# talmolab/sleap-nn

Hardware: AMD Instinct MI355X
Metric: frames/sec bottom-up UNet 1024x1024 inference (higher is better)
Workload: dtype f32

## Files before the change

sleap_nn_amd/csrc/model.hip:

```cpp
#include <algorithm>
#include <atomic>
#include <cmath>
#include <cstring>
#include <mutex>
#include <type_traits>
#include <vector>

#include "model_internal.h"
#include "train_kernels.h"

static constexpr size_t PH_PROBE_WORDS_PER_OP = 32768;

namespace ph {

static thread_local std::string g_err;

void set_error(const char* fmt, ...) {
  char buf[1024];
  va_list ap;
  va_start(ap, fmt);
  vsnprintf(buf, sizeof(buf), fmt, ap);
  va_end(ap);
  g_err = buf;
}
// ... 1174 lines not shown
        a.coutp = pad16(d.cout);
        a.B = batch;
        a.H = s0.h;
        a.W = s0.w;
        a.relu = (d.flags & PH_FLAG_RELU) ? 1 : 0;
        a.bn = op.bn;
        a.clock_probe = m->clock_probe ? m->clock_probe + PH_PROBE_WORDS_PER_OP * (op_index - 1) : nullptr;
        a.dst_pool = d.dst2 >= 0 ? slot_ptr(d.dst2) : nullptr;
        a.skip_dst = (a.dst_pool && plan.reuse && !plan.unread.empty() && plan.unread[d.dst]) ? 1 : 0;
        a.wpack_dma = op.w_dma_dev;
        a.wpack_wino = op.w_wino_dev;
        a.wpack_wino2 = op.w_wino2_dev;
        a.wpack_w16 = op.w_w16_dev;
        a.w16 = op.w16_dev;
        a.zeros = m->zeros_dev;
        apply_conv_options(m, a);
        a.wpack_sm = op.w_sm_dev;
        a.use_sm = m->conv_smallmap >= 2 ? 2 : ((m->conv_smallmap == 1 && m->conv_splitk == 1 && plan.reuse && m->use_dma) ? 1 : 0);
        a.wpack_wino4 = op.w_wino4_dev;
        a.use_wino4 = m->conv_wino4 == 3 ? 2 : ((m->conv_wino4 == 2 || (m->conv_wino4 == 1 && plan.reuse)) ? 1 : 0);
        if (op.w_n64_dev && op.w_wino2_dev && op.w_wino_dev && (m->conv_n32_wino2d >= 2 || (m->conv_n32_wino2d == 1 && plan.reuse)) && m->use_dma && m->conv_wino && m->conv_wino2d && m->conv_persist && !w16_fits(a) && wino2d_fits(a)) {
          a.bn = 64;
          a.wpack = op.w_n64_dev;
          a.bias = op.b_n64_dev;
          a.wpack_dma = nullptr;
        }
        if (a.splitk == 1 && !plan.reuse) a.splitk = 0;
        if (plan.tmp_bytes > 0) {
          a.split_scratch = reinterpret_cast<float*>(ws + plan.tmp_offset);
          a.split_scratch_bytes = plan.tmp_bytes;
        }
        if (deferred_up >= 0) {
          const ph_op_desc& up = m->ops[deferred_up].d;
          const SlotShape& sl = plan.slots[up.src0];
          ConvArgs f = a;
          f.src1 = slot_ptr(up.src0);
          f.src1_lowres = 1;
          if ((m->use_dma && conv3x3_dma_is_wino4(f)) || conv3x3_takes_sm(f)) {
            a = f;
          } else {
            rc = launch_upsample(slot_ptr(up.src0), slot_ptr(up.dst), batch, sl.h, sl.w, sl.cp, s);
            if (rc != PH_OK) return rc;
          }
          deferred_up = -1;
        }
        const bool on_sm = conv3x3_takes_sm(a);
        const double fill = (double)s0.h * s0.w / ((double)((s0.h + 15) / 16 * 16) * ((s0.w + 31) / 32 * 32));
        const double n_fill = (double)a.coutp / ((a.coutp + op.bn - 1) / op.bn * op.bn);
        const int bn_g = op.bn_g > 0 ? op.bn_g : 128;
        const double n_fill_g = (double)a.coutp / ((a.coutp + bn_g - 1) / bn_g * bn_g);
        double halo_gain = (op.w_wino_dev && m->use_dma) ? m->gemm_fill_threshold / m->gemm_fill_threshold_wino : 1.0;
        double halo_fill = fill;
        if (m->use_dma && m->conv_wino && m->conv_wino2d && m->conv_persist && op.w_wino2_dev && a.bn == 64 && a.c0p + a.c1p >= 32 && wino2d_fits(a)) {
          halo_fill = (double)s0.h * s0.w / ((double)((s0.h + 15) / 16 * 16) * ((s0.w + 15) / 16 * 16));
          halo_gain = m->gemm_fill_threshold / m->gemm_fill_threshold_wino2d;
        }
        if (!on_sm && m->use_dma && d.dst2 < 0 && op.w_gemm_dev && !a.src1_lowres && (halo_fill * halo_gain < m->gemm_fill_threshold || n_fill * halo_fill * halo_gain < 0.8 * n_fill_g)) {
          GemmArgs g{};
          g.src0 = a.src0;
          g.src1 = a.src1;
          g.c0p = a.c0p;
          g.c1p = a.c1p;
          g.wpack = op.w_gemm_dev;
          g.bias = op.b_gemm_dev;
          g.dst = a.dst;
          g.zeros = m->zeros_dev;
          g.coutp = a.coutp;
          g.bn = op.bn_g;
          g.M = batch * s0.h * s0.w;
          g.mode = 2;
          g.H = s0.h;
          g.W = s0.w;
          g.act = a.relu ? 1 : 0;
          g.late_split = m->gemm_late_split;
          g.persist2 = m->gemm_persist2;
          kv[op_index - 1] = PH_KV_ROWGEMM;
          rc = launch_gemm(g, s);
          break;
        }
        if (m->head_fuse && !a.dst_pool && ((a.coutp == 64 && a.bn == 64) || ((a.coutp == 16 || a.coutp == 32) && a.bn == 32)) && m->use_dma) {
          for (size_t j = op_index; j < m->ops.size(); ++j) {
            const ph_op_desc& hx = m->ops[j].d;
            if (hx.kind != PH_OP_HEAD || hx.src0 != d.dst) continue;
            ConvArgs no4 = a;
            no4.use_wino4 = 0;
            const bool on_w2d = a.coutp == 64 && hx.cout <= 32 && pad16(hx.cin0) == 64 && conv3x3_dma_is_wino2d(no4) && wino2d_ksplit(no4) <= 1;
            const bool on_w16 = a.coutp <= 32 && hx.cout <= 16 && pad16(hx.cin0) == a.coutp && conv3x3_dma_is_w16_head(a);
            const bool sm_head = on_sm && a.coutp <= 32 && pad16(hx.cin0) == a.coutp;
            if (!(hx.flags & PH_FLAG_SOFTMAX) && out_dev[hx.out_index] && (sm_head || (!on_sm && (on_w2d || on_w16)))) {
              a.head_w = m->ops[j].w_dev;
              a.head_b = m->ops[j].b_dev;
              a.head_dst = out_dev[hx.out_index];
              a.head_cout = hx.cout;
              a.head_wcp = a.coutp;
              a.head_sigmoid = (hx.flags & PH_FLAG_SIGMOID) ? 1 : 0;
              head_done[j] = 1;
              if (plan.reuse) {
                bool other = false;
                for (size_t k = 0; k < m->ops.size(); ++k)
                  if (k != j && (m->ops[k].d.src0 == d.dst || m->ops[k].d.src1 == d.dst)) other = true;
                if (!other) a.skip_dst = 1;
              }
            }
            break;
          }
        }
        if (m->pool_peephole && !a.dst_pool && !a.head_w && a.relu && m->use_dma && (a.bn == 64 || m->dma32) && op_index < m->ops.size()) {
          const ph_op_desc& nx = m->ops[op_index].d;
          if (nx.kind == PH_OP_POOL && nx.src0 == d.dst) {
            a.dst_pool = slot_ptr(nx.dst);
            if (conv3x3_dma_is_f2x2(a))
              pooled_by_conv = d.dst;
            else
              a.dst_pool = nullptr;
          }
        }
        if (on_sm) {
          kv[op_index - 1] = PH_KV_SMALLMAP;
          rc = launch_conv3x3_sm(a, s);
          break;
        }
        kv[op_index - 1] = (m->use_dma && (a.bn == 64 || m->dma32)) ? conv3x3_dma_variant(a) : PH_KV_DIRECT;
        rc = (m->use_dma && (a.bn == 64 || m->dma32)) ? launch_conv3x3_dma(a, s) : launch_conv3x3(a, s);
        break;
      }
      case PH_OP_POOL: {
        if (pooled_by_conv == d.src0) {
          pooled_by_conv = -1;
          break;
        }
        const SlotShape& s0 = plan.slots[d.src0];
        rc = fmt == FMT_F32 ? launch_pool(slot_ptr(d.src0), slot_ptr(d.dst), batch, s0.h, s0.w, s0.cp, s)
                            : launch_pool_fmt(fmt, slot_ptr(d.src0), slot_ptr(d.dst), batch, s0.h, s0.w, s0.cp, s);
        break;
      }
      case PH_OP_UPSAMPLE: {
        const SlotShape& s0 = plan.slots[d.src0];
        if (fmt == FMT_F32 && plan.reuse && m->upsample_fold && (m->conv_wino4 || m->conv_smallmap) && m->use_dma && op_index < m->ops.size()) {
          const PackedOp& nxo = m->ops[op_index];
          const ph_op_desc& nx = nxo.d;
          bool only = nx.kind == PH_OP_CONV && nx.ksize == 3 && nx.src1 == d.dst && nx.src0 != d.dst && nx.dst2 < 0 && ((m->conv_wino4 && nxo.w_wino4_dev != nullptr) || (m->conv_smallmap && nxo.w_sm_dev != nullptr));
          for (size_t k = 0; only && k < m->ops.size(); ++k)
            if (k != op_index && (m->ops[k].d.src0 == d.dst || m->ops[k].d.src1 == d.dst)) only = false;
          if (only) {
            deferred_up = (int)op_index - 1;
            break;
          }
        }
        if (fmt == FMT_F16 && plan.reuse && m->upsample_fold && m->conv_f16_rows && op_index < m->ops.size()) {
          const PackedOp& nxo = m->ops[op_index];
          const ph_op_desc& nx = nxo.d;
          bool only = nx.kind == PH_OP_CONV && nx.ksize == 3 && nx.src1 == d.dst && nx.src0 != d.dst && nxo.bn == 64 && plan.slots[nx.src0].h == 2 * s0.h && plan.slots[nx.src0].w == 2 * s0.w;
          for (size_t k = 0; only && k < m->ops.size(); ++k)
            if (k != op_index && (m->ops[k].d.src0 == d.dst || m->ops[k].d.src1 == d.dst)) only = false;
          if (only) {
            deferred_up = (int)op_index - 1;
            break;
          }
        }
        rc = fmt == FMT_F32 ? launch_upsample(slot_ptr(d.src0), slot_ptr(d.dst), batch, s0.h, s0.w, s0.cp, s)
                            : launch_upsample_fmt(fmt, slot_ptr(d.src0), slot_ptr(d.dst), batch, s0.h, s0.w, s0.cp, s, (fmt == FMT_F16 && m->upsample_f16math) ? 1 : 0);
        break;
      }
      case PH_OP_CONVT: {
        const SlotShape& s0 = plan.slots[d.src0];
        PH_REQUIRE(s0.c == d.cin0, "convT channel mismatch");
        if (fmt == FMT_F32 && m->convt_phase && op.wt_phase_dev[0]) {
          const SlotShape& so = plan.slots[d.dst];
          for (int ph = 0; ph < (m->convt_one_launch ? 1 : 4) && rc == PH_OK; ++ph) {
            GemmArgs g{};
            g.src0 = slot_ptr(d.src0);
            g.c0p = s0.cp;
// ... 448 lines not shown
```

sleap_nn_amd/csrc/net_kernels.hip:

```cpp
#include <type_traits>

#include "act_format.h"
#include "common.h"
#include "net_kernels.h"
#include "f16_kernels.h"

namespace ph {

typedef float f32x16 __attribute__((ext_vector_type(16)));
typedef float f32x4 __attribute__((ext_vector_type(4)));

constexpr int TH = 8, TW = 32, KC = 16, LROW = 20;
constexpr int HALO_W = TW + 2, HALO_H = TH + 2;

__device__ __forceinline__ void deal_tile(int id, int tiles, int nt_count, int* tile, int* ntile) {
  if ((tiles & 7) == 0) {
    const int xcd = id & 7, j = id >> 3;
    *ntile = j % nt_count;
    *tile = xcd * (tiles >> 3) + j / nt_count;
  } else {
    *ntile = id % nt_count;
    *tile = id / nt_count;
  }
}
// ... 1128 lines not shown
        if (a.accumulate) v += *d;
        *d = v;
      }
    }
    __syncthreads();
  }
}

static int cu_count(int* out);
static int launch_conv3x3_c16(const ConvArgs& a, hipStream_t s) {
  int n_cu = 0;
  const int rc = cu_count(&n_cu);
  if (rc != PH_OK) return rc;
  const int tiles = ((a.W + C16_TW - 1) / C16_TW) * ((a.H + C16_TH - 1) / C16_TH) * a.B;
  hipLaunchKernelGGL(conv3x3_c16_kernel, dim3(std::min(tiles, n_cu * 4)), dim3(256), 0, s, a);
  PH_HIP_CHECK(hipGetLastError());
  return PH_OK;
}

static int cu_count(int* out) { return device_cu_count(out); }

static int conv3x3_dma_route(const ConvArgs& a) {
  const bool wino = a.use_wino && a.wpack_wino && (a.bn == 64 || a.use_wino != 2);
  if (wino && a.persist && a.use_wino4 && a.c0p + a.c1p >= a.wino4_min_cin && wino4_fits(a)) return 4;
  if (wino && a.persist && a.use_w16 && w16_fits(a)) return 1;
  if (a.use_c16 && a.w16 && a.c0p == 16 && a.coutp == 16 && !a.src1 && !a.dst_pool) return 0;
  if (wino && a.persist && a.use_wino2d && a.wpack_wino2 && a.bn == 64 && a.c0p + a.c1p >= 32 && wino2d_fits(a)) return 2;
  return 3;
}
bool conv3x3_takes_sm(const ConvArgs& a) {
  if (!a.use_sm || !sm_fits(a)) return false;
  if (a.use_sm >= 2) return true;
  int n_cu = 0;
  if (device_cu_count(&n_cu) != PH_OK || n_cu <= 0) n_cu = 256;
  ConvArgs hi = a;
  hi.src1_lowres = 0;
  const int r = a.src1_lowres && conv3x3_dma_route(a) == 4 ? 4 : conv3x3_dma_route(hi);
  const double extra = (a.src1_lowres && r != 4) ? 6.0 : 0.0;
  const double Qn = (a.c0p + a.c1p) / 4.0;
  const long ntc = (a.coutp + 63) / 64;
  const bool may_split = a.split_scratch != nullptr;
  double other;
  if (r == 4) {
    const int ks = may_split ? wino4_ksplit_shape(a.B, a.H, a.W, a.c0p + a.c1p, a.coutp, a.splitk, n_cu) : 1;
    const long t4 = (long)((a.H + 15) / 16) * ((a.W + 31) / 32) * a.B * ntc;
    other = (double)((t4 * ks + n_cu - 1) / n_cu) * (11.0 + 1.5 * Qn / ks) + (ks > 1 ? 8.0 : 0.0);
  } else if (r == 2) {
    const int ks = may_split ? wino2d_ksplit_shape(a.B, a.H, a.W, a.c0p + a.c1p, a.coutp, a.splitk, n_cu) : 1;
    const long t2 = (long)((a.H + 15) / 16) * ((a.W + 15) / 16) * a.B * ntc;
    other = (double)((t2 * ks + n_cu - 1) / n_cu) * (8.0 + 1.0 * Qn / ks) + (ks > 1 ? 8.0 : 0.0);
  } else if (r == 1) {
    const long t1 = (long)((a.H + 31) / 32) * ((a.W + 15) / 16) * a.B;
    other = (double)((t1 + n_cu - 1) / n_cu) * (6.0 + 3.0 * (a.c0p + a.c1p) / 16.0);
  } else {
    return false;
  }
  if ((r == 4 || r == 2) && (a.coutp & 63) != 0 && (a.coutp & 63) <= 32) other *= 0.6;
  return sm_cost_us(a, n_cu) < other + extra;
}
bool conv3x3_dma_honours_mask(const ConvArgs& a) {
  const int r = conv3x3_dma_route(a);
  return (r == 1 || r == 2 || r == 4) && !a.dst_pool && !a.head_w && !a.skip_dst;
}
bool conv3x3_dma_is_f2x2(const ConvArgs& a) { const int r = conv3x3_dma_route(a); return r == 1 || r == 2; }
bool conv3x3_dma_is_wino2d(const ConvArgs& a) { return conv3x3_dma_route(a) == 2; }
bool conv3x3_dma_is_wino4(const ConvArgs& a) { return conv3x3_dma_route(a) == 4; }
bool conv3x3_dma_is_w16_head(const ConvArgs& a) { return conv3x3_dma_route(a) == 1 && w16_takes_head(a); }
int conv3x3_dma_variant(const ConvArgs& a) {
  switch (conv3x3_dma_route(a)) {
    case 0: return PH_KV_C16;
    case 1: return PH_KV_W16;
    case 2: return wino2d_ksplit(a) > 1 ? PH_KV_WINO2D_KS : PH_KV_WINO2D;
    case 4: return PH_KV_WINO4;
    default: break;
  }
  const bool wino = a.use_wino && a.wpack_wino && (a.bn == 64 || a.use_wino != 2);
  return (a.persist && wino) ? PH_KV_WINO1D : PH_KV_DIRECT;
}

int launch_conv3x3_dma(const ConvArgs& a, hipStream_t s) {
  const int route = conv3x3_dma_route(a);
  PH_REQUIRE(!a.relu_mask_src || ((route == 1 || route == 2 || route == 4) && !a.dst_pool && !a.head_w && !a.skip_dst),
             "relu_mask_src is applied by the F(2x2,3x3) / F(4x4,3x3) kernels' plain stores only (ask conv3x3_dma_honours_mask first)");
  PH_REQUIRE(!a.head_w || (route == 2 && !a.dst_pool && a.coutp == 64 && a.bn == 64 && a.head_cout >= 1 && a.head_cout <= 32 && a.head_wcp == 64 && a.head_b && a.head_dst) ||
                 (route == 1 && w16_takes_head(a) && a.head_cout >= 1 && a.head_cout <= 16 && a.head_wcp == a.coutp && a.head_b && a.head_dst),
             "a fused head needs the F(2x2,3x3) kernel on 64 output channels (<= 32 head channels) or the wave-private kernel on 16 -> 16 / 32 -> 32 channels (<= 16 head channels): ask conv3x3_dma_is_wino2d / _is_w16_head first");
  if (route == 1) return launch_conv3x3_w16(a, s);
  if (route == 0) return launch_conv3x3_c16(a, s);
  if (route == 2) return launch_conv3x3_wino2d(a, s);
  if (route == 4) return launch_conv3x3_wino4(a, s);
  PH_REQUIRE(!a.src1_lowres, "a half-resolution second source is only taken by the F(4x4,3x3) kernel (ask conv3x3_dma_is_wino4 first)");
  const int tiles = ((a.W + TW - 1) / TW) * ((a.H + D_TH - 1) / D_TH) * a.B;
  const int ntc = (a.coutp + a.bn - 1) / a.bn;
  const bool wino = a.use_wino && a.wpack_wino && (a.bn == 64 || a.use_wino != 2);
  int n_cu = 0;
  if (a.persist) {
    const int rc = cu_count(&n_cu);
    if (rc != PH_OK) return rc;
  }
  const dim3 grid_p(std::min(tiles * ntc, n_cu)), grid_1(tiles * ntc);
  const size_t lds_w = (size_t)(2 * D_A_PIECES + 3 * 12 * (a.bn / 32)) * 1024;
  const size_t lds_d = (size_t)2 * (D_A_PIECES + 9 * a.bn / 16) * 1024;
  if (a.bn == 64) {
    if (a.persist && wino)
      hipLaunchKernelGGL((conv3x3_wino_persist_kernel<64, 8>), grid_p, dim3(512), lds_w, s, a);
    else if (a.persist)
      hipLaunchKernelGGL(conv3x3_mfma_dma_persist_kernel<64>, grid_p, dim3(512), lds_d, s, a);
    else
      hipLaunchKernelGGL(conv3x3_mfma_dma_kernel<64>, grid_1, dim3(512), lds_d, s, a);
  } else {
    if (a.persist && wino)
      hipLaunchKernelGGL((conv3x3_wino_persist_kernel<32, 8>), grid_p, dim3(512), lds_w, s, a);
    else if (a.persist)
      hipLaunchKernelGGL(conv3x3_mfma_dma_persist_kernel<32>, grid_p, dim3(512), lds_d, s, a);
    else
      hipLaunchKernelGGL(conv3x3_mfma_dma_kernel<32>, grid_1, dim3(512), lds_d, s, a);
  }
  PH_HIP_CHECK(hipGetLastError());
  return PH_OK;
}

__device__ __forceinline__ void stem_store(const StemArgs& a, void* base, size_t pix, int c, float v) {
  if (a.out_fmt == FMT_SPLIT)
    store1<FMT_SPLIT>(base, pix, 16, c, v);
  else if (a.out_fmt == FMT_F16) {
    store1<FMT_F16>(base, pix, 32, c, v);
    store1<FMT_F16>(base, pix, 32, c + 16, 0.f);
  } else
    store1<FMT_F32>(base, pix, 16, c, v);
}

__device__ __forceinline__ void stem_store4(const StemArgs& a, void* base, size_t pix, int c0, const float (&v)[4]) {
  if (a.out_fmt == FMT_SPLIT)
    store4<FMT_SPLIT>(base, pix, 16, c0, v);
  else if (a.out_fmt == FMT_F16) {
    const float z[4] = {0.f, 0.f, 0.f, 0.f};
    store4<FMT_F16>(base, pix, 32, c0, v);
    store4<FMT_F16>(base, pix, 32, c0 + 16, z);
  } else
    store4<FMT_F32>(base, pix, 16, c0, v);
}

template <int CIN, int WINO>
__global__ __launch_bounds__(256, (CIN == 1 && WINO == 2) ? 5 : 4) void stem_fused_kernel(StemArgs a) {
  constexpr int IMG_W = TW + 4, IMG_H = TH + 4;
  __shared__ __attribute__((aligned(16))) float sA[HALO_H * HALO_W * LROW];
  __shared__ float sImg[CIN * IMG_H * IMG_W];
  __shared__ float sW0[9 * CIN * 16 + 16];

  const int tid = threadIdx.x;
  const int lane = tid & 63, wave = tid >> 6;
  const int tiles_x = (a.W + TW - 1) / TW, tiles_y = (a.H + TH - 1) / TH;
  const int per_xcd = (tiles_x * tiles_y * a.B + 7) >> 3;
  int t = (blockIdx.x & 7) * per_xcd + (blockIdx.x >> 3);
  if (t >= tiles_x * tiles_y * a.B) return;
  const int tx = t % tiles_x;
  t /= tiles_x;
  const int ty = t % tiles_y;
  const int b = t / tiles_y;
  const int x0 = tx * TW, y0 = ty * TH;

  for (int i = tid; i < CIN * IMG_H * IMG_W; i += 256) {
    const int c = i / (IMG_H * IMG_W), r = i - c * (IMG_H * IMG_W);
    const int iy = r / IMG_W, ix = r - iy * IMG_W;
    const int gy = y0 + iy - 2, gx = x0 + ix - 2;
    float v = 0.f;
    if (gy >= 0 && gy < a.H && gx >= 0 && gx < a.W) {
      const size_t o = (((size_t)b * CIN + c) * a.H + gy) * a.W + gx;
      if (a.dtype == 0)
// ... 629 lines not shown
```

sleap_nn_amd/csrc/wino4_kernels.hip:

```cpp
#include <type_traits>

#include "common.h"
#include "net_kernels.h"

#ifndef W4_EXP
#define W4_EXP 0
#endif

namespace ph {

typedef float f32x16 __attribute__((ext_vector_type(16)));
typedef float f32x4 __attribute__((ext_vector_type(4)));
typedef float f32x2 __attribute__((ext_vector_type(2)));

constexpr int W4_TX = 8, W4_TY = 4;
constexpr int W4_PW = 4 * W4_TX;
constexpr int W4_PH = 4 * W4_TY;
constexpr int W4_RAW_FLOATS = 12 * 256;
constexpr int W4_V_FLOATS = 36 * 128;
constexpr int W4_LDS_FLOATS = 36 * 1024;
constexpr int W4_Q_FLOATS = 36 * 64 * 4;
constexpr int P4_WAVE_FLOATS = 4 * 256 + 128;

__device__ __forceinline__ float wino4_g_row(int k, float g0, float g1, float g2) {
  switch (k) {
    case 0: return 0.25f * g0;
    case 1: return (-1.f / 6.f) * ((g0 + g2) + g1);
    case 2: return (-1.f / 6.f) * ((g0 + g2) - g1);
    case 3: return (1.f / 24.f) * g0 + ((1.f / 12.f) * g1 + (1.f / 6.f) * g2);
    case 4: return (1.f / 24.f) * g0 + ((-1.f / 12.f) * g1 + (1.f / 6.f) * g2);
    default: return g2;
  }
}
__global__ __launch_bounds__(256) void wino4_pack_kernel(const float* __restrict__ src, float* __restrict__ dst, int ntiles, int nchunks) {
  __shared__ float unit[W4_Q_FLOATS];
  const int quarter = blockIdx.x % (4 * nchunks), ntile = blockIdx.x / (4 * nchunks);
  const int tid = threadIdx.x;
  const int row = tid >> 2, kcl = tid & 3;
  const int nt = row >> 5, lx = row & 31, lh = kcl >> 1, j = kcl & 1;
  const float* w = src + (((size_t)ntile * nchunks + (quarter >> 2)) * 9 * 64 + row) * 16 + (quarter & 3) * 4 + kcl;
  const size_t ts = (size_t)64 * 16;
  float g[9];
#pragma unroll
  for (int t = 0; t < 9; ++t) g[t] = w[t * ts];
#pragma unroll
  for (int xi = 0; xi < 6; ++xi) {
    float h[3];
#pragma unroll
    for (int kx = 0; kx < 3; ++kx) h[kx] = wino4_g_row(xi, g[0 * 3 + kx], g[1 * 3 + kx], g[2 * 3 + kx]);
#pragma unroll
    for (int nu = 0; nu < 6; ++nu) {
      const float u = wino4_g_row(nu, h[0], h[1], h[2]);
      const int p = xi * 6 + nu, pgp = p / 9, pl = p % 9;
      unit[(nt * 4 + pgp) * P4_WAVE_FLOATS + (pl < 8 ? (((pl >> 1) * 64 + lh * 32 + lx) << 2) + j * 2 + (pl & 1) : 1024 + ((lh * 32 + lx) << 1) + j)] = u;
    }
  }
  __syncthreads();
  float* out = dst + (size_t)blockIdx.x * W4_Q_FLOATS;
#pragma unroll 4
  for (int i = tid; i < W4_Q_FLOATS; i += 256) out[i] = unit[i];
}
int64_t wino4_pack_floats(int ntiles, int nchunks) { return (int64_t)ntiles * 4 * nchunks * W4_Q_FLOATS; }
int launch_wino4_pack(const float* wpack, float* wino, int ntiles, int nchunks, hipStream_t s) {
  hipLaunchKernelGGL(wino4_pack_kernel, dim3((unsigned)(ntiles * 4 * nchunks)), dim3(256), 0, s, wpack, wino, ntiles, nchunks);
  PH_HIP_CHECK(hipGetLastError());
  return PH_OK;
}

__device__ __forceinline__ void w4_deal_tile(int id, int tiles, int nt_count, int rot, int* tile, int* ntile) {
  if ((tiles & 7) == 0) {
    const int xcd = id & 7, j = id >> 3;
    *ntile = (j % nt_count + rot) % nt_count;
    *tile = xcd * (tiles >> 3) + j / nt_count;
  } else {
    *ntile = (id % nt_count + rot) % nt_count;
    *tile = id / nt_count;
  }
}

__device__ __forceinline__ void w4_col_pass(const float (&t)[6], float (&v)[6]) {
  const float a = fmaf(-4.f, t[2], t[4]);
  const float b = fmaf(-4.f, t[1], t[3]);
  const float c = t[4] - t[2];
  const float d0 = t[3] - t[1];
  const float d = d0 + d0;
  v[0] = fmaf(4.f, t[0], fmaf(-5.f, t[2], t[4]));
  v[1] = a + b;
  v[2] = a - b;
  v[3] = c + d;
  v[4] = c - d;
  v[5] = fmaf(4.f, t[1], fmaf(-5.f, t[3], t[5]));
}

template <int P, int N>
__device__ __forceinline__ void p4_vput(float* slot, int vwq, int vwd, const float* v) {
  if constexpr (N > 0) {
    constexpr int pgc = P / 9, pl = P % 9;
    if constexpr (pl == 8) {
      slot[pgc * P4_WAVE_FLOATS + vwd] = v[0];
      p4_vput<P + 1, N - 1>(slot, vwq, vwd, v + 1);
    } else if constexpr ((pl & 1) == 0 && N >= 2) {
      *reinterpret_cast<float2*>(slot + pgc * P4_WAVE_FLOATS + (pl >> 1) * 256 + vwq) = make_float2(v[0], v[1]);
      p4_vput<P + 2, N - 2>(slot, vwq, vwd, v + 2);
    } else {
      slot[pgc * P4_WAVE_FLOATS + (pl >> 1) * 256 + vwq + (pl & 1)] = v[0];
      p4_vput<P + 1, N - 1>(slot, vwq, vwd, v + 1);
    }
  }
}

template <bool LOWRES, bool KS = false>
__global__ __launch_bounds__(512) void conv3x3_wino4_kernel(ConvArgs a) {
  extern __shared__ __attribute__((aligned(16))) float lds[];
  const int tid = threadIdx.x;
  const int lane = tid & 63;
  const int pw = __builtin_amdgcn_readfirstlane(tid >> 6);
  const int nt = pw >> 2, pg = pw & 3;
  const int lx = lane & 31, lh = lane >> 5;
  const int xg = pw < 4 ? (pw >> 1) : 2 + ((pw - 4) >> 1);
  const int typ = 2 * (pw & 1) + (lane >> 5), txp = (lane >> 2) & 7, cp = lane & 3;

  const int tiles_x = (a.W + W4_PW - 1) / W4_PW;
  const int tiles_y = (a.H + W4_PH - 1) / W4_PH;
  const int tiles = tiles_x * tiles_y * a.B;
  const int ntc = (a.coutp + 63) / 64;
  const int units = tiles * ntc;
  const int total = KS ? units * a.ksplit : units;
  const int Q0 = a.c0p / 4, Q1 = a.c1p / 4, Q = Q0 + Q1;
  constexpr int lowres = LOWRES ? 1 : 0;
  const int Hl = a.H >> 1, Wl = a.W >> 1;

#ifdef W4_CLOCK
  const unsigned long long clk_c0 = __builtin_amdgcn_s_memtime(), clk_r0 = __builtin_amdgcn_s_memrealtime();
#endif
  float* const rawbuf = lds;
  float* const vbuf = lds + 2 * W4_RAW_FLOATS;

  const float alpha = xg == 0 ? -4.f : -1.f, beta = xg == 0 ? 1.f : 2.f, nbeta = -beta;
  const int pbase_f = ((4 * typ + (xg == 2 ? 0 : 1)) * 36 + txp) * 4 + cp;
  const int pbase_l = ((2 * typ) * 18 + txp) * 4 + cp;
  const int vwq = ((cp >> 1) * 32 + typ * 8 + txp) * 4 + (cp & 1) * 2;
  const int vwd = 1024 + ((cp >> 1) * 32 + typ * 8 + txp) * 2 + (cp & 1);
  const int vrq = pg * P4_WAVE_FLOATS + lane * 4, vrd = pg * P4_WAVE_FLOATS + 1024 + lane * 2;

  struct Plan {
    int b, x0, y0, ntile;
  };
  const int G = (int)gridDim.x;
  const bool rotate = (a.coutp & 63) != 0 && (a.coutp & 63) <= 32 && ntc > 1 && (((tiles & 7) == 0) ? ((G & 7) == 0 && (G >> 3) % ntc == 0) : (G % ntc == 0));
  auto setup = [&](int vid, Plan& P) {
    int t, ntile;
    w4_deal_tile(vid, tiles, ntc, rotate ? vid / G : 0, &t, &ntile);
    const int tx = t % tiles_x;
    t /= tiles_x;
    const int ty = t % tiles_y;
    P.b = t / tiles_y;
    P.x0 = tx * W4_PW;
    P.y0 = ty * W4_PH;
    P.ntile = ntile;
  };

  const __amdgpu_buffer_rsrc_t wrsrc = __builtin_amdgcn_make_buffer_rsrc((void*)a.wpack_wino4, 0, (int)((unsigned)ntc * (unsigned)Q * (unsigned)(W4_Q_FLOATS * 4)), 0x00020000);
  const unsigned w_lane = (unsigned)(pw * P4_WAVE_FLOATS + lane * 4) * 4u;
  const unsigned w_lane9 = (unsigned)(pw * P4_WAVE_FLOATS + 1024 + lane * 2) * 4u;

  for (int vid = blockIdx.x; vid < total; vid += gridDim.x) {
#ifdef W4_STAMP
    const unsigned long long tile_t0 = __builtin_amdgcn_s_memtime();
#endif
    Plan P;
    const int ksl = KS ? vid / units : 0;
    const int qbeg = KS ? ksl * Q / a.ksplit : 0;
    const int qend = KS ? (ksl + 1) * Q / a.ksplit : Q;
    setup(KS ? vid - ksl * units : vid, P);
    unsigned off0[2], off1[2];
#pragma unroll
    for (int i = 0; i < 2; ++i) {
      const int e = (pw + 8 * i) * 64 + lane;
      const int hy = e / 36, rem = e - hy * 36;
      const int pl = rem / 9, k = rem - pl * 9;
      const int hx = 4 * k + pl;
      const int gy = P.y0 + hy - 1, gx = P.x0 + hx - 1;
      const bool in = pw + 8 * i < 11 && hy < W4_PH + 2 && hx < W4_PW + 2 && gy >= 0 && gy < a.H && gx >= 0 && gx < a.W;
      off0[i] = in ? (unsigned)((P.b * a.H + gy) * a.W + gx) * (unsigned)(a.c0p * 4) : 0xFFFFFF00u;
      if (!lowres) {
        off1[i] = (in && a.c1p > 0) ? (unsigned)((P.b * a.H + gy) * a.W + gx) * (unsigned)(a.c1p * 4) : 0xFFFFFF00u;
      } else {
        const int ly = e / 18, rem2 = e - ly * 18;
        const int par = rem2 / 9, kk = rem2 - par * 9;
        const int lc = 2 * kk + par;
        const int sy = min(max((P.y0 >> 1) - 1 + ly, 0), Hl - 1), sx = min(max((P.x0 >> 1) - 1 + lc, 0), Wl - 1);
        off1[i] = (ly < W4_PH / 2 + 2) ? (unsigned)((P.b * Hl + sy) * Wl + sx) * (unsigned)(a.c1p * 4) : 0xFFFFFF00u;
      }
    }
    const __amdgpu_buffer_rsrc_t rsrc0 = __builtin_amdgcn_make_buffer_rsrc((void*)a.src0, 0, (int)((unsigned)(a.B * a.H * a.W) * (unsigned)(a.c0p * 4)), 0x00020000);
// ... 291 lines not shown
          acc[2] = P4_MFMA(wf[1][2], vf1[2], acc[2]);
          acc[3] = P4_MFMA(wf[1][3], vf1[3], acc[3]);
          load_w(q + 1, 1);
        }
        P4_SB
        P4_ST(6)
        if constexpr (MM) {
          acc[4] = P4_MFMA(wf[2][0], vf2[0], acc[4]);
          acc[5] = P4_MFMA(wf[2][1], vf2[1], acc[5]);
          vf9 = *reinterpret_cast<const float2*>(vd);
        }
        if constexpr (PAIR) t_cols(xg_tag, lr_tag, second, vslot);
        if constexpr (MM) {
          acc[4] = P4_MFMA(wf[2][2], vf2[2], acc[4]);
          acc[5] = P4_MFMA(wf[2][3], vf2[3], acc[5]);
          load_w(q + 1, 2);
        }
        P4_SB
        P4_ST(7)
        asm volatile("s_waitcnt lgkmcnt(0)" ::: "memory");
        if (!(W4_EXP & 4)) __builtin_amdgcn_s_barrier();
        P4_SB
        P4_ST_END
      }
    };
    auto run = [&](auto xg_tag, auto mm_tag) __attribute__((always_inline)) {
      if constexpr (LOWRES) {
        const int qs = min(max(Q0 - 1, qbeg), qend);
        quarters(xg_tag, mm_tag, std::false_type{}, qbeg, qs);
        quarters(xg_tag, mm_tag, std::true_type{}, qs, qend);
      } else {
        quarters(xg_tag, mm_tag, std::false_type{}, qbeg, qend);
      }
    };
    auto run_mm = [&](auto mm_tag) __attribute__((always_inline)) {
      switch (xg) {
        case 0: run(std::integral_constant<int, 0>{}, mm_tag); break;
        case 1: run(std::integral_constant<int, 1>{}, mm_tag); break;
        case 2: run(std::integral_constant<int, 2>{}, mm_tag); break;
        default: run(std::integral_constant<int, 3>{}, mm_tag); break;
      }
    };
    if (nt == 1 && P.ntile * 64 + 32 >= a.coutp) {
      run_mm(std::false_type{});
    } else {
      run_mm(std::true_type{});
      acc[6] = P4_MFMA(wf[3][0], vf3[0], acc[6]);
      acc[7] = P4_MFMA(wf[3][1], vf3[1], acc[7]);
      acc[8] = P4_MFMA(wf9[0], vf9.x, acc[8]);
      acc[6] = P4_MFMA(wf[3][2], vf3[2], acc[6]);
      acc[7] = P4_MFMA(wf[3][3], vf3[3], acc[7]);
      acc[8] = P4_MFMA(wf9[1], vf9.y, acc[8]);
    }

#ifdef W4_STAMP
    const unsigned long long tile_t2 = __builtin_amdgcn_s_memtime();
#endif
    float* const exch = lds;
    auto dump = [&](int r) __attribute__((always_inline)) {
      int d0 = ((pg * 9 * 32 + lx) * 8 + ((nt * 4 + lh) ^ (lx & 7))) << 2;
      asm volatile("" : "+v"(d0));
#pragma unroll
      for (int kk = 0; kk < 2; ++kk) {
        float* const dk = exch + (d0 ^ (kk << 3));
#pragma unroll
        for (int i = 0; i < 9; ++i) {
          f32x4 v;
          if (r == 0) {
            v[0] = acc[i][4 * kk + 0];
            v[1] = acc[i][4 * kk + 1];
            v[2] = acc[i][4 * kk + 2];
            v[3] = acc[i][4 * kk + 3];
          } else {
            v[0] = acc[i][8 + 4 * kk + 0];
            v[1] = acc[i][8 + 4 * kk + 1];
            v[2] = acc[i][8 + 4 * kk + 2];
            v[3] = acc[i][8 + 4 * kk + 3];
          }
          *reinterpret_cast<f32x4*>(dk + i * 1024) = v;
        }
      }
      asm volatile("s_waitcnt lgkmcnt(0)" ::: "memory");
    };
    auto finish = [&](int round) __attribute__((always_inline)) {
      const int tile = tid >> 4, cq = (tid >> 1) & 7, hc = tid & 1;
      const int ty = tile >> 3, tx = tile & 7;
      int z0 = ((tile * 8 + (cq ^ (tile & 7))) << 2) + 2 * hc;
      asm volatile("" : "+v"(z0));
      const float* zp = exch + z0;
      f32x2 z[4][6];
#pragma unroll
      for (int n = 0; n < 6; ++n) {
        f32x2 m[6];
#pragma unroll
        for (int x = 0; x < 6; ++x) m[x] = *reinterpret_cast<const f32x2*>(zp + (x * 6 + n) * 1024);
#pragma unroll
        for (int e = 0; e < 2; ++e) {
          const float s12 = m[1][e] + m[2][e], d12 = m[1][e] - m[2][e], s34 = m[3][e] + m[4][e], d34 = m[3][e] - m[4][e];
          z[0][n][e] = (m[0][e] + s12) + s34;
          z[1][n][e] = fmaf(2.f, d34, d12);
          z[2][n][e] = fmaf(4.f, s34, s12);
          z[3][n][e] = fmaf(8.f, d34, d12) + m[5][e];
        }
      }
      const int co = P.ntile * 64 + (cq >> 2) * 32 + round * 16 + (cq & 3) * 4 + 2 * hc;
      const f32x2 bias = KS ? f32x2{0.f, 0.f} : *reinterpret_cast<const f32x2*>(a.bias + co);
      const int oy0 = P.y0 + 4 * ty, ox = P.x0 + 4 * tx;
      const bool live = oy0 < a.H && ox < a.W && co < a.coutp;
      f32x2 prow[2];
#pragma unroll
      for (int aa = 0; aa < 4; ++aa) {
        const f32x2 s12 = z[aa][1] + z[aa][2], d12 = z[aa][1] - z[aa][2], s34 = z[aa][3] + z[aa][4], d34 = z[aa][3] - z[aa][4];
        f32x2 y[4];
        y[0] = ((z[aa][0] + s12) + s34) + bias;
        y[1] = (d12 + 2.f * d34) + bias;
        y[2] = (s12 + 4.f * s34) + bias;
        y[3] = ((d12 + 8.f * d34) + z[aa][5]) + bias;
        if (live) {
          float* const dp = a.dst + ((size_t)(P.b * a.H + oy0 + aa) * a.W + ox) * a.coutp + co + (KS ? (size_t)ksl * a.split_stride : (size_t)0);
#pragma unroll
          for (int bb = 0; bb < 4; ++bb) {
            f32x2 v = y[bb];
            if (a.relu) {
#pragma unroll
              for (int e = 0; e < 2; ++e) v[e] = fmaxf(v[e], 0.f);
            }
            if (a.relu_mask_src) {
              const f32x2 f = *reinterpret_cast<const f32x2*>(a.relu_mask_src + (dp - a.dst) + (size_t)bb * a.coutp);
#pragma unroll
              for (int e = 0; e < 2; ++e) v[e] = f[e] > 0.f ? v[e] : 0.f;
            }
            y[bb] = v;
            if ((KS || !a.skip_dst) && !(W4_EXP & 512)) *reinterpret_cast<f32x2*>(dp + (size_t)bb * a.coutp) = v;
          }
          if (!KS && a.dst_pool) {
            f32x2 m0, m1;
#pragma unroll
            for (int e = 0; e < 2; ++e) {
              m0[e] = fmaxf(y[0][e], y[1][e]);
              m1[e] = fmaxf(y[2][e], y[3][e]);
            }
            if (aa & 1) {
#pragma unroll
              for (int e = 0; e < 2; ++e) {
                m0[e] = fmaxf(m0[e], prow[0][e]);
                m1[e] = fmaxf(m1[e], prow[1][e]);
              }
              float* const pp = a.dst_pool + ((size_t)(P.b * (a.H >> 1) + ((oy0 + aa) >> 1)) * (a.W >> 1) + (ox >> 1)) * a.coutp + co;
              *reinterpret_cast<f32x2*>(pp) = m0;
              *reinterpret_cast<f32x2*>(pp + a.coutp) = m1;
            } else {
              prow[0] = m0;
              prow[1] = m1;
            }
          }
        }
      }
      asm volatile("s_waitcnt lgkmcnt(0)" ::: "memory");
    };
#ifdef W4_STAMP
    unsigned long long e1 = 0, e2 = 0, e3 = 0;
#define P4_ET(x) x = __builtin_amdgcn_s_memtime();
#else
#define P4_ET(x)
#endif
    dump(0);
    __builtin_amdgcn_s_barrier();
    P4_ET(e1)
    finish(0);
    __builtin_amdgcn_s_barrier();
    P4_ET(e2)
    dump(1);
    __builtin_amdgcn_s_barrier();
    P4_ET(e3)
    finish(1);
    __builtin_amdgcn_s_barrier();
#ifdef W4_STAMP
    if (a.clock_probe && lane == 0 && vid == (int)blockIdx.x) {
      unsigned long long* o = a.clock_probe + ((size_t)blockIdx.x * 12 + pw) * 8;
#ifdef W4_STTILE
      o[0] = (tile_t1 - tile_t0) * (unsigned long long)(qend - qbeg);
      o[1] = st[0] + st[1] + st[2] + st[3] + st[4] + st[5] + st[6] + st[7];
      o[2] = (e1 - tile_t2) * (unsigned long long)(qend - qbeg);
      o[3] = (e2 - e1) * (unsigned long long)(qend - qbeg);
      o[4] = (e3 - e2) * (unsigned long long)(qend - qbeg);
      o[5] = (__builtin_amdgcn_s_memtime() - e3) * (unsigned long long)(qend - qbeg);
      o[6] = o[7] = 0;
#else
#pragma unroll
      for (int i = 0; i < 8; ++i) o[i] = st[i];
#endif
    }
#endif
  }
#ifdef W4_CLOCK
  if (a.clock_probe && tid == 0) {
    a.clock_probe[blockIdx.x * 2] = __builtin_amdgcn_s_memtime() - clk_c0;
    a.clock_probe[blockIdx.x * 2 + 1] = __builtin_amdgcn_s_memrealtime() - clk_r0;
  }
#endif
}

int prepare_wino4_kernels() {
  hipError_t e = hipSuccess;
  if (e == hipSuccess) e = hipFuncSetAttribute(reinterpret_cast<const void*>(conv3x3_wino4_kernel<false, false>), hipFuncAttributeMaxDynamicSharedMemorySize, W4_LDS_FLOATS * (int)sizeof(float));
  if (e == hipSuccess) e = hipFuncSetAttribute(reinterpret_cast<const void*>(conv3x3_wino4_kernel<true, false>), hipFuncAttributeMaxDynamicSharedMemorySize, W4_LDS_FLOATS * (int)sizeof(float));
  if (e == hipSuccess) e = hipFuncSetAttribute(reinterpret_cast<const void*>(conv3x3_wino4_kernel<false, true>), hipFuncAttributeMaxDynamicSharedMemorySize, W4_LDS_FLOATS * (int)sizeof(float));
  if (e == hipSuccess) e = hipFuncSetAttribute(reinterpret_cast<const void*>(conv3x3_wino4_kernel<true, true>), hipFuncAttributeMaxDynamicSharedMemorySize, W4_LDS_FLOATS * (int)sizeof(float));
  if (e != hipSuccess) {
    set_error("hipFuncSetAttribute(wino4) failed: %s", hipGetErrorString(e));
    return PH_E_HIP;
  }
  return PH_OK;
}

bool wino4_fits(const ConvArgs& a) {
  if (!a.wpack_wino4 || a.bn != 64 || (a.H & 3) || (a.W & 3) || a.head_w || a.accumulate) return false;
  if (a.src1_lowres && (!a.src1 || (a.H & 1) || (a.W & 1))) return false;
  const uint64_t px = (uint64_t)a.B * a.H * a.W;
  if (px * (uint64_t)a.c0p * 4 >= 0xFFFFFF00ull || px * (uint64_t)a.c1p * 4 >= 0xFFFFFF00ull || px >= 0x7FFFFFFFull) return false;
  const uint64_t wbytes = (uint64_t)((a.coutp + 63) / 64) * (uint64_t)((a.c0p + a.c1p) / 4) * W4_Q_FLOATS * 4;
  if (wbytes >= 0xFFFFFF00ull) return false;
  if (a.use_wino4 >= 2) return true;
  int n_cu = 0;
  if (device_cu_count(&n_cu) != PH_OK || n_cu <= 0) n_cu = 256;
  const bool may_split = a.split_scratch != nullptr;
  const int ks4 = may_split ? wino4_ksplit_shape(a.B, a.H, a.W, a.c0p + a.c1p, a.coutp, a.splitk, n_cu) : 1;
  const int ks2 = may_split ? wino2d_ksplit_shape(a.B, a.H, a.W, a.c0p + a.c1p, a.coutp, a.splitk, n_cu) : 1;
  const long ntc = (a.coutp + 63) / 64;
  const long t4 = (long)((a.H + W4_PH - 1) / W4_PH) * ((a.W + W4_PW - 1) / W4_PW) * a.B * ntc;
  const long t2 = (long)((a.H + 15) / 16) * ((a.W + 15) / 16) * a.B * ntc;
  const double Qn = (a.c0p + a.c1p) / 4.0;
  const double cost4 = (double)((t4 * ks4 + n_cu - 1) / n_cu) * (11.0 + 1.5 * Qn / ks4) + (ks4 > 1 ? 8.0 : 0.0);
  const double cost2 = (double)((t2 * ks2 + n_cu - 1) / n_cu) * (8.0 + 1.0 * Qn / ks2) + (ks2 > 1 ? 8.0 : 0.0);
  return cost4 <= cost2;
}

int wino4_ksplit_shape(int B, int H, int W, int cinp, int coutp, int splitk, int n_cu) {
  if (splitk <= 0 || cinp < 128) return 1;
  const long units = (long)((H + W4_PH - 1) / W4_PH) * ((W + W4_PW - 1) / W4_PW) * B * ((coutp + 63) / 64);
  const int q = cinp / 4;
  if (splitk >= 2) return std::max(1, std::min(splitk, q / 4));
  if (units * 2 > n_cu) return 1;
  return (int)std::max<long>(1, std::min<long>(n_cu / units, q / 16));
}
int64_t wino4_split_scratch_bytes(int B, int H, int W, int cinp, int coutp, int splitk, int n_cu) {
  if ((H & 3) || (W & 3)) return 0;
  const int ks = wino4_ksplit_shape(B, H, W, cinp, coutp, splitk, n_cu);
  return ks > 1 ? (int64_t)ks * B * H * W * coutp * 4 : 0;
}
static int wino4_ksplit(const ConvArgs& a) {
  if (!a.split_scratch || a.relu_mask_src) return 1;
  int n_cu = 0;
  if (device_cu_count(&n_cu) != PH_OK || n_cu <= 0) return 1;
  const int ks = wino4_ksplit_shape(a.B, a.H, a.W, a.c0p + a.c1p, a.coutp, a.splitk, n_cu);
  return (ks > 1 && (int64_t)ks * a.B * a.H * a.W * a.coutp * 4 <= a.split_scratch_bytes) ? ks : 1;
}

int launch_conv3x3_wino4(const ConvArgs& a, hipStream_t s) {
  PH_REQUIRE(wino4_fits(a), "wino4: N tile 64, H and W multiples of 4, no fused head / accumulate, tensors below 4 GiB");
  int n_cu = 0;
  const int rc = device_cu_count(&n_cu);
  if (rc != PH_OK) return rc;
  const int tiles = ((a.W + W4_PW - 1) / W4_PW) * ((a.H + W4_PH - 1) / W4_PH) * a.B;
  const int ntc = (a.coutp + 63) / 64;
  const int ksplit = wino4_ksplit(a);
  if (ksplit > 1) {
    ConvArgs k = a;
    k.dst = a.split_scratch;
    k.relu = 0;
    k.dst_pool = nullptr;
    k.skip_dst = 0;
    k.ksplit = ksplit;
    k.split_stride = (long long)a.B * a.H * a.W * a.coutp;
    const dim3 grid(std::min(tiles * ntc * ksplit, n_cu));
    if (a.src1_lowres)
      hipLaunchKernelGGL((conv3x3_wino4_kernel<true, true>), grid, dim3(512), (size_t)W4_LDS_FLOATS * sizeof(float), s, k);
    else
      hipLaunchKernelGGL((conv3x3_wino4_kernel<false, true>), grid, dim3(512), (size_t)W4_LDS_FLOATS * sizeof(float), s, k);
    PH_HIP_CHECK(hipGetLastError());
    return launch_splitk_reduce(a.split_scratch, k.split_stride, ksplit, a.bias, a.skip_dst ? nullptr : a.dst, a.dst_pool, a.B, a.H, a.W, a.coutp, a.relu, s);
  }
  if (a.src1_lowres)
    hipLaunchKernelGGL((conv3x3_wino4_kernel<true, false>), dim3(std::min(tiles * ntc, n_cu)), dim3(512), (size_t)W4_LDS_FLOATS * sizeof(float), s, a);
  else
    hipLaunchKernelGGL((conv3x3_wino4_kernel<false, false>), dim3(std::min(tiles * ntc, n_cu)), dim3(512), (size_t)W4_LDS_FLOATS * sizeof(float), s, a);
  PH_HIP_CHECK(hipGetLastError());
  return PH_OK;
}

}
```

Baseline: 2992.

## Fuse 1x1 output head into the F(4x4,3x3) Winograd conv kernel

Adds a head-fused variant of the wino4 convolution kernel. After each output round it stages the ReLU'd tile in LDS and runs a small MFMA 1x1 head matmul, writing sigmoid/bias head outputs directly. The model planner now lets wino4 take the head instead of falling back to the F(2x2) kernel. The goal is to avoid a separate head launch and a reread of the 64-channel activation, and to keep the faster wino4 route for the last decoder conv. The cost is extra barriers and LDS traffic inside the kernel. The skip_dst path may also drop the full-resolution store.

```diff
diff --git a/sleap_nn_amd/csrc/model.hip b/sleap_nn_amd/csrc/model.hip
--- a/sleap_nn_amd/csrc/model.hip
+++ b/sleap_nn_amd/csrc/model.hip
@@ -1280,12 +1280,17 @@
           for (size_t j = op_index; j < m->ops.size(); ++j) {
             const ph_op_desc& hx = m->ops[j].d;
             if (hx.kind != PH_OP_HEAD || hx.src0 != d.dst) continue;
-            ConvArgs no4 = a;
-            no4.use_wino4 = 0;
-            const bool on_w2d = a.coutp == 64 && hx.cout <= 32 && pad16(hx.cin0) == 64 && conv3x3_dma_is_wino2d(no4) && wino2d_ksplit(no4) <= 1;
+            ConvArgs h4 = a;
+            h4.head_w = m->ops[j].w_dev;
+            h4.head_b = m->ops[j].b_dev;
+            h4.head_dst = out_dev[hx.out_index];
+            h4.head_cout = hx.cout;
+            h4.head_wcp = pad16(hx.cin0);
+            const bool on_w4 = a.coutp == 64 && out_dev[hx.out_index] && conv3x3_dma_is_wino4(a) && conv3x3_dma_is_wino4(h4);
+            const bool on_w2d = a.coutp == 64 && hx.cout <= 32 && pad16(hx.cin0) == 64 && conv3x3_dma_is_wino2d(a) && wino2d_ksplit(a) <= 1;
             const bool on_w16 = a.coutp <= 32 && hx.cout <= 16 && pad16(hx.cin0) == a.coutp && conv3x3_dma_is_w16_head(a);
             const bool sm_head = on_sm && a.coutp <= 32 && pad16(hx.cin0) == a.coutp;
-            if (!(hx.flags & PH_FLAG_SOFTMAX) && out_dev[hx.out_index] && (sm_head || (!on_sm && (on_w2d || on_w16)))) {
+            if (!(hx.flags & PH_FLAG_SOFTMAX) && out_dev[hx.out_index] && (sm_head || (!on_sm && (on_w4 || on_w2d || on_w16)))) {
               a.head_w = m->ops[j].w_dev;
               a.head_b = m->ops[j].b_dev;
               a.head_dst = out_dev[hx.out_index];
diff --git a/sleap_nn_amd/csrc/net_kernels.hip b/sleap_nn_amd/csrc/net_kernels.hip
--- a/sleap_nn_amd/csrc/net_kernels.hip
+++ b/sleap_nn_amd/csrc/net_kernels.hip
@@ -1234,9 +1234,9 @@
   const int route = conv3x3_dma_route(a);
   PH_REQUIRE(!a.relu_mask_src || ((route == 1 || route == 2 || route == 4) && !a.dst_pool && !a.head_w && !a.skip_dst),
              "relu_mask_src is applied by the F(2x2,3x3) / F(4x4,3x3) kernels' plain stores only (ask conv3x3_dma_honours_mask first)");
-  PH_REQUIRE(!a.head_w || (route == 2 && !a.dst_pool && a.coutp == 64 && a.bn == 64 && a.head_cout >= 1 && a.head_cout <= 32 && a.head_wcp == 64 && a.head_b && a.head_dst) ||
+  PH_REQUIRE(!a.head_w || route == 4  || (route == 2 && !a.dst_pool && a.coutp == 64 && a.bn == 64 && a.head_cout >= 1 && a.head_cout <= 32 && a.head_wcp == 64 && a.head_b && a.head_dst) ||
                  (route == 1 && w16_takes_head(a) && a.head_cout >= 1 && a.head_cout <= 16 && a.head_wcp == a.coutp && a.head_b && a.head_dst),
-             "a fused head needs the F(2x2,3x3) kernel on 64 output channels (<= 32 head channels) or the wave-private kernel on 16 -> 16 / 32 -> 32 channels (<= 16 head channels): ask conv3x3_dma_is_wino2d / _is_w16_head first");
+             "a fused head needs the F(2x2,3x3) kernel on 64 output channels (<= 32 head channels), the F(4x4,3x3) kernel on 64 output channels (<= 16 head channels) or the wave-private kernel on 16 -> 16 / 32 -> 32 channels (<= 16 head channels): ask conv3x3_dma_is_wino2d / _is_wino4 / _is_w16_head first");
   if (route == 1) return launch_conv3x3_w16(a, s);
   if (route == 0) return launch_conv3x3_c16(a, s);
   if (route == 2) return launch_conv3x3_wino2d(a, s);
diff --git a/sleap_nn_amd/csrc/wino4_kernels.hip b/sleap_nn_amd/csrc/wino4_kernels.hip
--- a/sleap_nn_amd/csrc/wino4_kernels.hip
+++ b/sleap_nn_amd/csrc/wino4_kernels.hip
@@ -20,6 +20,8 @@
 constexpr int W4_V_FLOATS = 36 * 128;
 constexpr int W4_LDS_FLOATS = 36 * 1024;
 constexpr int W4_Q_FLOATS = 36 * 64 * 4;
+constexpr int W4_HEAD_MAX = 16;
+constexpr int W4_HS_TILE = 16 * 32 + 32;
 constexpr int P4_WAVE_FLOATS = 4 * 256 + 128;
 
 __device__ __forceinline__ float wino4_g_row(int k, float g0, float g1, float g2) {
@@ -109,8 +111,9 @@
   }
 }
 
-template <bool LOWRES, bool KS = false>
-__global__ __launch_bounds__(512) void conv3x3_wino4_kernel(ConvArgs a) {
+template <bool LOWRES, bool KS, bool HEAD>
+__device__ __forceinline__ void wino4_body(const ConvArgs& a) {
+  static_assert(!HEAD || (!KS && !LOWRES), "a fused head needs the whole K sum; only the full-resolution form is routed");
   extern __shared__ __attribute__((aligned(16))) float lds[];
   const int tid = threadIdx.x;
   const int lane = tid & 63;
@@ -568,6 +571,7 @@
       }
       asm volatile("s_waitcnt lgkmcnt(0)" ::: "memory");
     };
+    f32x4 hw0, hw1, hacc[4];
     auto finish = [&](int round) __attribute__((always_inline)) {
       const int tile = tid >> 4, cq = (tid >> 1) & 7, hc = tid & 1;
       const int ty = tile >> 3, tx = tile & 7;
@@ -589,6 +593,18 @@
           z[3][n][e] = fmaf(8.f, d34, d12) + m[5][e];
         }
       }
+      int cqo = cq;
+      if constexpr (HEAD) {
+        asm volatile("s_waitcnt lgkmcnt(0)" : "+v"(cqo)::"memory");
+        __builtin_amdgcn_s_barrier();
+        const int o = lane & 15, g = lane >> 4;
+        hw0 = hw1 = f32x4{0.f, 0.f, 0.f, 0.f};
+        if (o < a.head_cout) {
+          const float* const wp = a.head_w + (size_t)o * 64 + (g >> 1) * 32 + round * 16 + (g & 1) * 8;
+          hw0 = *reinterpret_cast<const f32x4*>(wp);
+          hw1 = *reinterpret_cast<const f32x4*>(wp + 4);
+        }
+      }
       const int co = P.ntile * 64 + (cq >> 2) * 32 + round * 16 + (cq & 3) * 4 + 2 * hc;
       const f32x2 bias = KS ? f32x2{0.f, 0.f} : *reinterpret_cast<const f32x2*>(a.bias + co);
       const int oy0 = P.y0 + 4 * ty, ox = P.x0 + 4 * tx;
@@ -602,6 +618,18 @@
         y[1] = (d12 + 2.f * d34) + bias;
         y[2] = (s12 + 4.f * s34) + bias;
         y[3] = ((d12 + 8.f * d34) + z[aa][5]) + bias;
+        if constexpr (HEAD) {
+          float* const sp = exch + tile * W4_HS_TILE + aa * 4 * 32 + 2 * hc;
+#pragma unroll
+          for (int bb = 0; bb < 4; ++bb) {
+            f32x2 v = y[bb];
+            if (a.relu) {
+#pragma unroll
+              for (int e = 0; e < 2; ++e) v[e] = fmaxf(v[e], 0.f);
+            }
+            *reinterpret_cast<f32x2*>(sp + bb * 32 + ((cqo ^ ((aa * 4 + bb) & 7)) << 2)) = v;
+          }
+        }
         if (live) {
           float* const dp = a.dst + ((size_t)(P.b * a.H + oy0 + aa) * a.W + ox) * a.coutp + co + (KS ? (size_t)ksl * a.split_stride : (size_t)0);
 #pragma unroll
@@ -650,17 +678,68 @@
 #else
 #define P4_ET(x)
 #endif
+    auto head_mm = [&](int round) __attribute__((always_inline)) {
+      if constexpr (HEAD) {
+        int j = lane & 15;
+        const int g = lane >> 4;
+        asm volatile("" : "+v"(j));
+        const float* const sp = exch + pw * 4 * W4_HS_TILE + j * 32;
+        const int c0 = ((2 * g) ^ (j & 7)) << 2, c1 = ((2 * g + 1) ^ (j & 7)) << 2;
+        f32x4 b0[4], b1[4];
+#pragma unroll
+        for (int blk = 0; blk < 4; ++blk) {
+          b0[blk] = *reinterpret_cast<const f32x4*>(sp + blk * W4_HS_TILE + c0);
+          b1[blk] = *reinterpret_cast<const f32x4*>(sp + blk * W4_HS_TILE + c1);
+        }
+#pragma unroll
+        for (int blk = 0; blk < 4; ++blk) {
+          if (round == 0) hacc[blk] = f32x4{0.f, 0.f, 0.f, 0.f};
+#pragma unroll
+          for (int e = 0; e < 4; ++e) hacc[blk] = __builtin_amdgcn_mfma_f32_16x16x4f32(hw0[e], b0[blk][e], hacc[blk], 0, 0, 0);
+#pragma unroll
+          for (int e = 0; e < 4; ++e) hacc[blk] = __builtin_amdgcn_mfma_f32_16x16x4f32(hw1[e], b1[blk][e], hacc[blk], 0, 0, 0);
+        }
+        asm volatile("s_waitcnt lgkmcnt(0)" ::: "memory");
+        if (round == 1) {
+#pragma unroll
+          for (int blk = 0; blk < 4; ++blk) {
+            const int t = pw * 4 + blk;
+            const int ty0 = P.y0 + 4 * (t >> 3), tx0 = P.x0 + 4 * (t & 7);
+            if (ty0 < a.H && tx0 < a.W) {
+#pragma unroll
+              for (int r = 0; r < 4; ++r) {
+                int o = 4 * g + r;
+                asm volatile("" : "+v"(o));
+                if (o < a.head_cout) {
+                  float v = hacc[blk][r] + a.head_b[o];
+                  if (a.head_sigmoid) v = 1.f / (1.f + expf(-v));
+                  a.head_dst[(((size_t)P.b * a.head_cout + o) * a.H + ty0 + (j >> 2)) * a.W + tx0 + (j & 3)] = v;
+                }
+              }
+            }
+          }
+        }
+      }
+    };
     dump(0);
     __builtin_amdgcn_s_barrier();
     P4_ET(e1)
     finish(0);
     __builtin_amdgcn_s_barrier();
+    if constexpr (HEAD) {
+      head_mm(0);
+      __builtin_amdgcn_s_barrier();
+    }
     P4_ET(e2)
     dump(1);
     __builtin_amdgcn_s_barrier();
     P4_ET(e3)
     finish(1);
     __builtin_amdgcn_s_barrier();
+    if constexpr (HEAD) {
+      head_mm(1);
+      __builtin_amdgcn_s_barrier();
+    }
 #ifdef W4_STAMP
     if (a.clock_probe && lane == 0 && vid == (int)blockIdx.x) {
       unsigned long long* o = a.clock_probe + ((size_t)blockIdx.x * 12 + pw) * 8;
@@ -687,12 +766,19 @@
 #endif
 }
 
+template <bool LOWRES, bool KS = false>
+__global__ __launch_bounds__(512) void conv3x3_wino4_kernel(ConvArgs a) {
+  wino4_body<LOWRES, KS, false>(a);
+}
+__global__ __launch_bounds__(512) void conv3x3_wino4_head_kernel(ConvArgs a) { wino4_body<false, false, true>(a); }
+
 int prepare_wino4_kernels() {
   hipError_t e = hipSuccess;
   if (e == hipSuccess) e = hipFuncSetAttribute(reinterpret_cast<const void*>(conv3x3_wino4_kernel<false, false>), hipFuncAttributeMaxDynamicSharedMemorySize, W4_LDS_FLOATS * (int)sizeof(float));
   if (e == hipSuccess) e = hipFuncSetAttribute(reinterpret_cast<const void*>(conv3x3_wino4_kernel<true, false>), hipFuncAttributeMaxDynamicSharedMemorySize, W4_LDS_FLOATS * (int)sizeof(float));
   if (e == hipSuccess) e = hipFuncSetAttribute(reinterpret_cast<const void*>(conv3x3_wino4_kernel<false, true>), hipFuncAttributeMaxDynamicSharedMemorySize, W4_LDS_FLOATS * (int)sizeof(float));
   if (e == hipSuccess) e = hipFuncSetAttribute(reinterpret_cast<const void*>(conv3x3_wino4_kernel<true, true>), hipFuncAttributeMaxDynamicSharedMemorySize, W4_LDS_FLOATS * (int)sizeof(float));
+  if (e == hipSuccess) e = hipFuncSetAttribute(reinterpret_cast<const void*>(conv3x3_wino4_head_kernel), hipFuncAttributeMaxDynamicSharedMemorySize, W4_LDS_FLOATS * (int)sizeof(float));
   if (e != hipSuccess) {
     set_error("hipFuncSetAttribute(wino4) failed: %s", hipGetErrorString(e));
     return PH_E_HIP;
@@ -700,8 +786,12 @@
   return PH_OK;
 }
 
+static int wino4_ksplit(const ConvArgs& a);
 bool wino4_fits(const ConvArgs& a) {
-  if (!a.wpack_wino4 || a.bn != 64 || (a.H & 3) || (a.W & 3) || a.head_w || a.accumulate) return false;
+  if (!a.wpack_wino4 || a.bn != 64 || (a.H & 3) || (a.W & 3) || a.accumulate) return false;
+  if (a.head_w && (a.coutp != 64 || a.head_wcp != 64 || a.head_cout < 1 || a.head_cout > W4_HEAD_MAX || !a.head_b || !a.head_dst || a.src1_lowres || a.dst_pool || a.relu_mask_src ||
+                   wino4_ksplit(a) > 1))
+    return false;
   if (a.src1_lowres && (!a.src1 || (a.H & 1) || (a.W & 1))) return false;
   const uint64_t px = (uint64_t)a.B * a.H * a.W;
   if (px * (uint64_t)a.c0p * 4 >= 0xFFFFFF00ull || px * (uint64_t)a.c1p * 4 >= 0xFFFFFF00ull || px >= 0x7FFFFFFFull) return false;
@@ -744,7 +834,7 @@
 }
 
 int launch_conv3x3_wino4(const ConvArgs& a, hipStream_t s) {
-  PH_REQUIRE(wino4_fits(a), "wino4: N tile 64, H and W multiples of 4, no fused head / accumulate, tensors below 4 GiB");
+  PH_REQUIRE(wino4_fits(a), "wino4: N tile 64, H and W multiples of 4, no accumulate, tensors below 4 GiB; a fused head: 64 output channels, at most 16 head channels, no split K / pool / ReLU mask / half-resolution source");
   int n_cu = 0;
   const int rc = device_cu_count(&n_cu);
   if (rc != PH_OK) return rc;
@@ -767,7 +857,9 @@
     PH_HIP_CHECK(hipGetLastError());
     return launch_splitk_reduce(a.split_scratch, k.split_stride, ksplit, a.bias, a.skip_dst ? nullptr : a.dst, a.dst_pool, a.B, a.H, a.W, a.coutp, a.relu, s);
   }
-  if (a.src1_lowres)
+  if (a.head_w)
+    hipLaunchKernelGGL(conv3x3_wino4_head_kernel, dim3(std::min(tiles * ntc, n_cu)), dim3(512), (size_t)W4_LDS_FLOATS * sizeof(float), s, a);
+  else if (a.src1_lowres)
     hipLaunchKernelGGL((conv3x3_wino4_kernel<true, false>), dim3(std::min(tiles * ntc, n_cu)), dim3(512), (size_t)W4_LDS_FLOATS * sizeof(float), s, a);
   else
     hipLaunchKernelGGL((conv3x3_wino4_kernel<false, false>), dim3(std::min(tiles * ntc, n_cu)), dim3(512), (size_t)W4_LDS_FLOATS * sizeof(float), s, a);
```

Result: no change. 3021 (median of 6 runs) (+1.0%).
